# cheshmi/parsy_bench

Measured on AMD Instinct MI355X. Metric: Cholesky factorizations/sec (+ SpTRSV solves/sec), SuiteSparse SPD set, higher is better.
Workload: dtype f64; 1 GPU; flan-class stand-in (BASELINE.json configs[2] when flan: Flan_1565): grid (116, 116, 116) 27-point stencil, geometric nested dissection; n=1560896, nnz_A_lower=21491316, nsuper=81191, nnz_L=2044454227, xsize=2421483055, etree_levels=17, launches_per_factorization=357, parallelism=1 GPU

## Files before the change

### parsy_bench_amd/csrc/capi_exec.hip

```cpp
#include <hip/hip_runtime.h>

#include <chrono>
#include <cstdio>
#include <cstring>
#include <map>
#include <algorithm>
#include <mutex>
#include <string>
#include <tuple>
#include <vector>

#include "../../include/parsy_amd.h"
#include "errors.hpp"
#include "hip_check.hpp"
#include "dist.hpp"
#include "executor.hpp"
#include "inspector.hpp"
#include "plan_util.hpp"
#include "refine.hpp"
#include "schedule_digest.hpp"
#include "cond.hpp"
#include "eigs.hpp"
#include "feature_states.hpp"

// ... 445 lines not shown
    const parsy::Schedule& S = pl->S;
    int64_t n = 0;
    int li = 0;
    for (const parsy::Launch& l : S.chol) {
        if (l.kind != parsy::kLaunchDense) continue;
        for (int q = l.first; q < l.first + l.count; ++q, ++n)
            if (out && n < cap) {
                out[2 * n] = li;
                out[2 * n + 1] = S.big_tasks[(size_t)q].part;
            }
        ++li;
    }
    return n;
}

int64_t parsy_debug_launches(const parsy_plan* pl, int which, int32_t* out, int64_t cap) {
    if (!pl || which < 0 || which > 2) return -1;
    const parsy::Schedule& S = pl->S;
    const std::vector<parsy::Launch>& seq = which == 0 ? S.chol : which == 1 ? S.solve : S.bsolve;
    for (size_t i = 0; out && i < seq.size() && (int64_t)i < cap; ++i) {
        const parsy::Launch& l = seq[i];
        const int32_t row[parsy::kLaunchFields] = {l.kind, l.first, l.count, l.level, l.side, l.wait_level, l.form, l.rows_only,
                                                   l.ticket, l.lds_bytes, l.stage, l.width, l.width_class, l.task_first, l.task_count};
        std::copy(row, row + parsy::kLaunchFields, out + (size_t)parsy::kLaunchFields * i);
    }
    return (int64_t)seq.size();
}

int parsy_debug_schedule_digest(const parsy_plan* pl, int field, uint64_t* out, const char** name) {
    if (!pl) return -1;
// ... 469 lines not shown
```

### parsy_bench_amd/csrc/chol_kernels.hip

```cpp
#include <hip/hip_runtime.h>

#include <algorithm>

#include <climits>

#include "device_util.hpp"
#include "kernels.hpp"

namespace parsy {

static constexpr int kThreads = 256;
static constexpr int kLdSub = kSub + 1;

#ifdef PARSY_BIGSTAMPS
__device__ unsigned long long g_bigtrace[2 * 8 * 1024];
__device__ int g_bigstamp_cfg[2];
#define BIGSTAMP(i) do { if (st_on) g_bigtrace[((size_t)st_slot * 1024 + st_n) * 8 + (i)] = __builtin_readcyclecounter(); } while (0)
#else
#define BIGSTAMP(i) do { } while (0)
#endif

#ifdef PARSY_STAMPS
__device__ unsigned long long g_stamps[32];
#define STAMP(i) do { if (threadIdx.x == 0) g_stamps[i] = wall_clock64(); } while (0)
// ... 1354 lines not shown
static constexpr int kBigThreads = 64 * kBigWaves;
static_assert(kBK % 4 == 0 && kBK % kBigWaves == 0, "k_chol_big: a wave stages kBK / waves columns per operand");
struct BigLds {
    double R[2][kBK * kBLd];
    double C[2][kBK * kBLd];
};

static constexpr int kGldsAux = 0;
__device__ __forceinline__ void glds16(const double* g, double* lds) {
    __builtin_amdgcn_global_load_lds((const __attribute__((address_space(1))) void*)g,
                                     (__attribute__((address_space(3))) void*)lds, 16, 0, kGldsAux);
}

__global__ __launch_bounds__(kBigThreads, 4) void k_chol_big(const SnDesc* __restrict__ sn,
                                                             const int32_t* __restrict__ relpos,
                                                             const WaveEntry* __restrict__ ents,
                                                             const TileDesc* __restrict__ tasks,
                                                             double* __restrict__ L) {
    __shared__ __attribute__((aligned(16))) BigLds S;
    {
        int agpr_hint = 0;
        asm volatile("; accumulators in AGPRs %0" ::"a"(agpr_hint));
    }
    const int tid = threadIdx.x, lane = tid & 63;
    const int wave = __builtin_amdgcn_readfirstlane(tid >> 6);
    const int l15 = lane & 15, kq = lane >> 4;
    const TileDesc td = tasks[blockIdx.x];
    const SnDesc D = sn[td.sn];
    double* __restrict__ G = L + D.px;
    const int ld = D.ld;
    const int64_t e_begin = td.wp, e_end = td.sp;
    if (e_begin >= e_end) return;
#ifdef PARSY_BIGABL_ZEROOPS
    const long long zmask = td.part == 12345 ? -1ll : 0ll;
#endif
#ifdef PARSY_BIGSTAMPS
    const bool st_on = (int)gridDim.x == g_bigstamp_cfg[0] && (int)blockIdx.x == g_bigstamp_cfg[1] && lane == 0 &&
                       (wave == 0 || wave == 5);
    const int st_slot = wave == 0 ? 0 : 1;
    int st_n = 0;
#endif

    int64_t le = e_begin;
    int lk = 0;
    WaveEntry LE = ents[le];
    int offR = 0, offC = 0;
    auto enter = [&]() {
// ... 601 lines not shown
    (void)hipMemcpyFromSymbol(out, HIP_SYMBOL(g_trace), sizeof(unsigned long long) * 16 * 512);
}
extern "C" void parsy_debug_tilephase(unsigned long long* out, int reset) {
    (void)hipMemcpyFromSymbol(out, HIP_SYMBOL(g_tilephase), sizeof(unsigned long long) * 16);
    if (reset) {
        unsigned long long z[16] = {};
        (void)hipMemcpyToSymbol(HIP_SYMBOL(g_tilephase), z, sizeof(z));
    }
}
#endif

void launch_chol_big(const DevicePattern& P, int first, int count, double* L, hipStream_t stream) {
    if (count <= 0) return;
    witness_launch(kWCholBig);
    hipLaunchKernelGGL(k_chol_big, dim3(count), dim3(kBigThreads), 0, stream, P.csn, P.relpos, P.big_entries,
                       P.big_tasks + first, L);
}

void launch_chol_tiles(const DevicePattern& P, int first, int count, double* L, hipStream_t stream) {
    if (count <= 0) return;
    witness_launch(kWCholTiles);
    hipLaunchKernelGGL(k_chol_tiles, dim3(count), dim3(kThreads), 0, stream, P.csn, P.relpos, P.wave_entries,
                       P.wave_ptr, P.split_ranges, P.tile_scratch, P.tiles + first, L);
}

int chain_workgroups_per_cu() {
    int nb = 0;
    if (hipOccupancyMaxActiveBlocksPerMultiprocessor(&nb, k_chol_chain, kThreads, 0) != hipSuccess) return 0;
    return nb;
}

// ... 18 lines not shown
```

### parsy_bench_amd/csrc/executor.hip

```cpp
#include "executor.hpp"

#include <climits>
#include <cstdlib>
#include <cstring>
#include <stdexcept>

#include "cond.hpp"
#include "device_util.hpp"
#include "errors.hpp"
#include "hip_check.hpp"
#include "plan_fwd.hpp"
#include "plan_util.hpp"
#include "refine.hpp"
#include "feature_states.hpp"

namespace parsy {

const Schedule& plan_schedule(const parsy_plan* plan) { return plan->S; }

int check_plan(const parsy_plan* pl, const char* who, PlanNeeds needs) {
    const std::string w(who);
    if (pl->device < 0) return set_last_error(w + ": plan was built without a device (device < 0)"), -1;
    if (needs == kNeedsDevice) return 0;
    if (pl->solve_only) return set_last_error(w + ": plan was built from L's pattern only (no A pattern)"), -1;
// ... 119 lines not shown
    return dptr ? 0 : pool_failed(pool);
}

int plan_upload_launches(parsy_plan* pl) {
    if (pl->device < 0) return 0;
    PARSY_HIP(hipSetDevice(pl->device));
    pl->launches.clear();
    pl->levels_open = false;
    const Schedule& S = pl->S;
    if (upload(pl, S.small_list, pl->dp.small_list, true)) return -1;
    if (upload(pl, S.small_ranges, pl->dp.small_ranges, true)) return -1;
    if (upload(pl, S.solve_small_ranges, pl->dp.solve_small_ranges, true)) return -1;
    if (upload(pl, S.bsolve_ranges, pl->dp.bsolve_ranges, true)) return -1;
    if (upload(pl, S.tiles, pl->dp.tiles, true)) return -1;
    if (upload(pl, S.big_tasks, pl->dp.big_tasks, true)) return -1;
    if (upload(pl, S.solve_small_list, pl->dp.solve_small_list, true)) return -1;
    if (upload(pl, S.solve_panels, pl->dp.solve_panels, true)) return -1;
    if (upload(pl, S.solve_mtasks, pl->dp.solve_mtasks, true)) return -1;
    if (upload(pl, S.solve_fix_list, pl->dp.solve_fix_list, true)) return -1;
    if (upload(pl, S.solve_wide_list, pl->dp.solve_wide_list, true)) return -1;
    if (upload(pl, S.bsolve_blocks, pl->dp.bsolve_blocks, true)) return -1;
    if (upload(pl, S.bsolve_below, pl->dp.bsolve_below, true)) return -1;
    (void)pl->bpart.reset();
    pl->dp.bpart = nullptr;
    if (upload(pl, S.bsolve_pairs, pl->dp.bsolve_pairs, true)) return -1;
    if (upload(pl, S.sub_members, pl->dp.sub_members, true) || upload(pl, S.sub_trees, pl->dp.sub_trees, true) ||
        upload(pl, S.sub_slots, pl->dp.sub_slots, true) || upload(pl, S.sub_out_rows, pl->dp.sub_out_rows, true))
        return -1;
    pl->dp.sub_ntiers = (!S.sub_tiers.empty() && solve_sub_prepare(S.sub_max_slots) == 0) ? (int)S.sub_tiers.size() : 0;
    {
// ... 568 lines not shown
```

### parsy_bench_amd/csrc/kernels.hpp

```cpp
#pragma once
#include <hip/hip_runtime.h>

#include <cstdint>

#include "schedule.hpp"

namespace parsy {

constexpr int kPassLanes = 8;

struct SolveGates {
    int mrhs_min = 6;
    int chain_mrhs_min = 2;
    int bmrhs_min = 16;
    bool bmrhs_wide_only = true;
    int bchain_min_blocks = 128;
    int small_halves_min = 512;
    int sub_mrhs_min = 6;
    int xt_min = 16;
    bool xt_min_set = false;
    int wait_bias = 0;
    int sub_abl = 0;
};
SolveGates read_solve_gates();
// ... 55 lines not shown
    const UpdDesc* upd = nullptr;
    const int32_t* relpos = nullptr;
    const int64_t* a_dst = nullptr;
    const int32_t* rows = nullptr;
    const WaveEntry* wave_entries = nullptr;
    const int64_t* wave_ptr = nullptr;
    const int64_t* split_ranges = nullptr;
    double* tile_scratch = nullptr;
    const int32_t* small_list = nullptr;
    const int32_t* small_ranges = nullptr;
    const int32_t* solve_small_ranges = nullptr;
    const int32_t* bsolve_ranges = nullptr;
    const TileDesc* tiles = nullptr;
    const WaveEntry* big_entries = nullptr;
    const TileDesc* big_tasks = nullptr;
    const int32_t* solve_small_list = nullptr;
    const PanelDesc* solve_panels = nullptr;
    const PanelDesc* solve_mtasks = nullptr;
    const int32_t* solve_fix_list = nullptr;
    const int32_t* solve_wide_list = nullptr;
    const PanelDesc* bsolve_pairs = nullptr;
    const PanelDesc* bsolve_below = nullptr;
    double* bpart = nullptr;
    const PanelDesc* bsolve_blocks = nullptr;
    const SubMember* sub_members = nullptr;
    const SubTree* sub_trees = nullptr;
    const uint16_t* sub_slots = nullptr;
    const int32_t* sub_out_rows = nullptr;
    int sub_ntiers = 0;
    int* info = nullptr;
// ... 68 lines not shown
```

### parsy_bench_amd/csrc/schedule.cpp

```cpp
#include "schedule.hpp"

#include <cstdio>
#include <map>
#include <algorithm>
#include <queue>
#include <climits>
#include <cmath>
#include <cstdlib>
#include <cstdint>
#include <functional>
#include <stdexcept>
#include <string>

namespace parsy {

static inline int ceil_div(int a, int b) { return (a + b - 1) / b; }

static int env_int(const char* name, int dflt) {
    const char* v = std::getenv(name);
    if (!v || !*v) return dflt;
    return std::atoi(v);
}

static int find_subtrees(const std::vector<int>& parent, const std::vector<uint8_t>& eligible,
// ... 671 lines not shown
                                              (int32_t)(launch >> 1), (int32_t)((launch & 1) == 0), bigk[i].sr, bigk[i].sc,
                                              (int64_t)mid, (int32_t)std::min<int64_t>(dweight, INT32_MAX),
                                              (int32_t)std::min<int64_t>(dchunks, INT32_MAX), nstrips});
        i = j;
    }
}

}

void build_schedule(const PatternRef& P, const size_t* lC, const int* A2p, const int* A2i,
                    const uint8_t* active, Schedule& S, int compute_units) {
    S = Schedule();
    BuildState B;
    B.knobs = read_build_knobs();
    B.compute_units = compute_units;
    if (compute_units > 0) S.walker_batch = std::max(4, std::min(kWalkerBatch, compute_units / 2));
    describe_supernodes(P, lC, A2p, S);
    list_updates(P, lC, A2p, A2i, S, B);
    choose_sizes(S, B.knobs);
    cut_pieces(P, S, B);
    describe_updates(S, B);
    cut_subtrees(S, B);
    choose_super_tiles(S, B);
    build_wave_streams(S, B);
    collect_big_entries(S, B);
    build_big_tasks(S, B);
    build_launches(S, active);
}


struct LaunchKnobs {
    bool force_unfused;
    int big_group;
    int chain_split;
    int bsolve_below;
    bool sub_tier_min_trees_set;
    int sub_tier_min_trees;
    int solve_one;
};

static LaunchKnobs read_launch_knobs(const Schedule& S) {
    LaunchKnobs K{};
    const char* fu = std::getenv("PARSY_FORCE_UNFUSED");
    K.force_unfused = fu && fu[0] == '1';
    K.big_group = env_int("PARSY_BIG_GROUP", kBigGroup);
    K.chain_split = env_int("PARSY_CHAIN_SPLIT", S.update_flops >= kChainSplitAutoFlops ? 2 : 0);
    K.bsolve_below = env_int("PARSY_BSOLVE_BELOW", 1);
    K.sub_tier_min_trees_set = std::getenv("PARSY_SUB_TIER_MIN_TREES") != nullptr;
    K.sub_tier_min_trees = env_int("PARSY_SUB_TIER_MIN_TREES", kSubTierMinTrees);
    K.solve_one = env_int("PARSY_SOLVE_ONE", 1);
    return K;
}

static void build_solve_one(Schedule& S, const LaunchKnobs& K, bool sharded);

static bool append_sub_tier(Schedule& S, const std::vector<std::vector<int32_t>>& trees, int top_level, int max_slots) {
    const size_t members0 = S.sub_members.size(), trees0 = S.sub_trees.size(), slots0 = S.sub_slots.size(),
                 outs0 = S.sub_out_rows.size();
    auto drop = [&] {
        S.sub_members.resize(members0);
        S.sub_trees.resize(trees0);
        S.sub_slots.resize(slots0);
        S.sub_out_rows.resize(outs0);
        return false;
    };
// ... 204 lines not shown
    L.task_first = task_first;
    return L;
}
static Launch fixup_launch(int32_t count, int32_t level) {
    Launch L = main_launch(kLaunchSolveFixup, 0, level);
    L.count = count;
    return L;
}
static Launch back_block_launch(int32_t first, int32_t count, int32_t level, int32_t width_class) {
    Launch L = main_launch(kLaunchBackBlock, first, level);
    L.count = count;
    L.width_class = width_class;
    return L;
}

namespace {

using BigTaskList = std::vector<const Schedule::BigTask*>;

struct LaunchState {
    LaunchKnobs knobs;
    std::vector<Launch> early;
    std::vector<size_t> level_begin;
    std::vector<BigTaskList> big_next, big_push;
};

void reset_launch_lists(Schedule& S) {
    S.n_chain_launches = 0;
    S.n_solve_chain_launches = 0;
    S.n_solve_wide = 0;
    S.n_bpart_slots = 0;
    S.small_list.clear();
    S.small_ranges.clear();
    S.tiles.clear();
    S.big_tasks.clear();
    S.chol.clear();
    S.solve_small_list.clear();
    S.solve_small_ranges.clear();
    S.solve_panels.clear();
    S.solve_mtasks.clear();
    S.solve_fix_list.clear();
    S.solve_wide_list.clear();
    S.solve.clear();
    S.sub_members.clear();
    S.sub_trees.clear();
    S.sub_slots.clear();
    S.sub_out_rows.clear();
    S.sub_tiers.clear();
    S.sub_max_slots = 0;
    S.sub_cover_level = -1;
// ... 17 lines not shown
        S.bsolve_subtree_all = S.bsolve_subtree;
    }
    S.solve_subtree = S.solve_subtree_all;
    S.bsolve_subtree = S.bsolve_subtree_all;
    if (active)
        for (auto* sub : {&S.solve_subtree, &S.bsolve_subtree}) {
            const int count = sub == &S.solve_subtree ? S.n_solve_subtrees : S.n_bsolve_subtrees;
            std::vector<uint8_t> whole((size_t)std::max(count, 0), 1);
            for (int t = 0; t < ns; ++t)
                if ((*sub)[t] >= 0 && !S.active[t]) whole[(size_t)(*sub)[t]] = 0;
            for (int t = 0; t < ns; ++t)
                if ((*sub)[t] >= 0 && !whole[(size_t)(*sub)[t]]) (*sub)[t] = -1;
        }
}

Launch emit_big(Schedule& S, int big_group, const BigTaskList& all, Launch L, bool dense) {
    BigTaskList v;
    for (const Schedule::BigTask* b : all)
        if (dense ? b->em > b->e0 : b->e1 > b->em) v.push_back(b);
    if (v.empty()) return L;
    L.first = (int32_t)S.big_tasks.size();
    auto wt = [dense](const Schedule::BigTask* b) { return dense ? b->dweight : b->weight; };
    auto desc = [dense](const Schedule::BigTask* b) {
        return dense ? TileDesc{b->sn, b->row0, b->col0, b->dchunks | (b->strips > 0 ? kDenseStripTask : 0), b->e0, b->em}
                     : TileDesc{b->sn, b->row0, b->col0, 0, b->em, b->e1};
    };
    auto by_weight = [&](const Schedule::BigTask* a, const Schedule::BigTask* b) { return wt(a) > wt(b); };
    int g = big_group;
    const int per_task = v[0]->sr * v[0]->sc;
    while (g > 1 && (int64_t)v.size() * per_task < (int64_t)8 * kBigGroupsPerXcd * g * g) g /= 2;
    if (g < std::max(v[0]->sr, v[0]->sc)) g = 1;
    if (g <= 1) {
        std::stable_sort(v.begin(), v.end(), by_weight);
        for (const Schedule::BigTask* b : v) S.big_tasks.push_back(desc(b));
// ... 54 lines not shown
    }
    size_t len = 0;
    for (int x = 0; x < 8; ++x) len = std::max(len, seq[x].size());
    for (size_t s = 0; s < len; ++s)
        for (int x = 0; x < 8; ++x) {
            if (s < seq[x].size()) {
                S.big_tasks.push_back(desc(seq[x][s]));
            } else {
                S.big_tasks.push_back(TileDesc{0, 0, 0, 0, 0, 0});
            }
        }
    L.count = (int32_t)(8 * len);
    return L;
}

template <class Position, class Append>
int32_t subtree_ranges(const Schedule& S, const std::vector<int32_t>& subtree, int count, const std::vector<double>& cost,
                       Position&& position, Append&& append, std::vector<int32_t>& ranges, bool chol = false) {
    std::vector<std::vector<int32_t>> members((size_t)count);
    std::vector<double> total((size_t)count, 0.0);
    for (int t = 0; t < S.nsuper; ++t)
        if (subtree[t] >= 0 && (chol ? S.active_piece[S.piece0[t]] : S.active[t])) {
            members[(size_t)subtree[t]].push_back(t);
            total[(size_t)subtree[t]] += cost[t];
        }
    std::vector<int32_t> order;
    for (int k = 0; k < count; ++k)
        if (!members[(size_t)k].empty()) order.push_back(k);
    std::stable_sort(order.begin(), order.end(), [&](int a, int b) { return total[(size_t)a] > total[(size_t)b]; });
    for (int k : order) {
// ... 21 lines not shown
            [&](int32_t t) { add_small(S, S.piece0[t], L); }, S.small_ranges, true);
        if (L.count > 0) S.chol.push_back(L);
    }
    Launch L = small_launch((int32_t)S.small_list.size(), lev);
    for (int q = S.clevelPtr[lev]; q < S.clevelPtr[lev + 1]; ++q) {
        const int t = S.clevelSet[q];
        if (!S.active_piece[t] || S.chol_subtree[S.csn_real[t]] >= 0) continue;
        if (is_small(S.csn[t])) add_small(S, t, L);
        else tiled.push_back(t);
    }
    L.count = (int32_t)S.small_list.size() - L.first;
    if (L.count > 0) S.chol.push_back(L);
}

void push_next_launches(Schedule& S, LaunchState& LS, int lev) {
    const int g = LS.knobs.big_group;
    if (lev + 2 < S.cnlevels) {
        Launch Ld = emit_big(S, g, LS.big_push[lev], side_launch(kLaunchDense, 0, lev + 2, lev), true);
        if (Ld.count > 0) LS.early.push_back(Ld);
        Launch Lp = emit_big(S, g, LS.big_push[lev], side_launch(kLaunchBig, 0, lev + 2, lev), false);
        if (Lp.count > 0) LS.early.push_back(Lp);
    }
    if (lev > 0) {
        Launch Ld = emit_big(S, g, LS.big_next[lev - 1], main_launch(kLaunchDense, 0, lev), true);
        if (Ld.count > 0) S.chol.push_back(Ld);
        Launch Ln = emit_big(S, g, LS.big_next[lev - 1], main_launch(kLaunchBig, 0, lev), false);
        if (Ln.count > 0) S.chol.push_back(Ln);
    }
}

void tiles_launch(Schedule& S, LaunchState& LS, int lev, const std::vector<int>& tiled) {
    Launch Lt = side_launch(kLaunchTiles, (int32_t)S.tiles.size(), lev, lev - 2);
    std::vector<std::pair<int32_t, TileDesc>> wt;
    for (int t : tiled) {
        const SnDesc& T = S.csn[t];
        const int nbc = ceil_div(T.w, kTile), nbr = ceil_div(T.r, kTile);
        const int32_t* tw = &S.tile_w[S.sn_tw0[t]];
        for (int J = 0; J < nbc; ++J)
            for (int I = J; I < nbr; ++I) {
                const int32_t wgt = tw[((size_t)J * nbr + I) * 2];
                if (wgt <= 0) continue;
                const int64_t si = S.tile_split[S.sn_tw0[t] / 2 + (size_t)J * nbr + I];
                if (si < 0) {
// ... 948 lines not shown
            if (u < 0 || mi < 1 || mi > kBigTile || nj < 1 || nj > kBigTile || E.ia + mi + ms > S.upd[u].m || E.ja + nj + ns > S.upd[u].n1 ||
                ident != (S.upd[u].rel < 0) || S.level_of[S.upd_src[u]] != b.src_level) {
                fail("BIG entry " + std::to_string(e) + " of piece " + std::to_string(b.sn) + " has a bad window or source");
                continue;
            }
            auto rel_at = [&](int k) { return ident ? k : S.relpos[(size_t)S.upd[u].rel + k] - T.rbias; };
            if (rel_at(E.ia) / win_r != b.row0 / win_r || rel_at(E.ia + mi + ms - 1) / win_r != b.row0 / win_r ||
                rel_at(E.ja) / win_c != b.col0 / win_c || rel_at(E.ja + nj + ns - 1) / win_c != b.col0 / win_c)
                fail("BIG entry " + std::to_string(e) + " names rows outside its task's tile");
            covered[(size_t)u] += block_flops(E);
        }
    }
    {
        std::vector<int64_t> starts;
        std::vector<int64_t> dense_pos(S.big_all.size(), -1), ragged_pos(S.big_all.size(), -1);
        int64_t li = 0;
        for (const Launch& l : S.chol) {
            ++li;
            if (l.kind != kLaunchBig && l.kind != kLaunchDense) continue;
            const bool dense = l.kind == kLaunchDense;
            const bool side = l.side != 0;
            auto find_task = [&](int64_t e) -> const Schedule::BigTask* {
                auto it = std::upper_bound(S.big_all.begin(), S.big_all.end(), e,
                                           [](int64_t v, const Schedule::BigTask& b) { return v < b.e0; });
                if (it == S.big_all.begin()) return nullptr;
                --it;
                return e < it->e1 ? &*it : nullptr;
            };
            auto right_launch = [&](const Schedule::BigTask& b) {
                return side != (b.next != 0) && (side ? l.wait_level : l.level - 1) == b.src_level;
            };
            for (int q = l.first; q < l.first + l.count; ++q) {
                const TileDesc& td = S.big_tasks[(size_t)q];
                if (td.wp >= td.sp) {
                    if (td.wp != td.sp) fail("BIG launch task " + std::to_string(q) + " has a negative entry range");
                    continue;
                }
                const Schedule::BigTask* it = find_task(td.wp);
                const bool ok = it && (dense ? (it->e0 == td.wp && it->em == td.sp && (td.part & ~kDenseStripTask) == it->dchunks &&
                                                ((td.part & kDenseStripTask) != 0) == (it->strips > 0))
                                             : (it->em == td.wp && it->e1 == td.sp));
                if (!ok || it->sn != td.sn || it->row0 != td.row0 || it->col0 != td.col0) {
                    fail("BIG launch task " + std::to_string(q) + " is not a task of the plan");
                    continue;
                }
                if (!right_launch(*it)) fail("BIG launch task " + std::to_string(q) + " runs in the launch of another source level");
                (dense ? dense_pos : ragged_pos)[(size_t)(it - S.big_all.data())] = li;
                starts.push_back(td.wp);
            }
        }
        std::sort(starts.begin(), starts.end());
        if (std::adjacent_find(starts.begin(), starts.end()) != starts.end()) fail("a BIG task is launched twice");
        int64_t want = 0;
        for (size_t k = 0; k < S.big_all.size(); ++k) {
            const Schedule::BigTask& b = S.big_all[k];
            if (b.em < b.e0 || b.em > b.e1) fail("BIG task " + std::to_string(k) + " has a bad dense / ragged split");
            int64_t dch = 0;
            int32_t nst = 0;
            for (int64_t e = b.e0; e < b.em; ++e) {
                const WaveEntry& E = S.big_entries[(size_t)e];
                nst += big_strip_rows(E) || big_strip_cols(E);
                if (E.K < kDenseChunk) fail("BIG entry " + std::to_string(e) + " is filed as dense but is narrower than a chunk");
                dch += ceil_div(E.K, kDenseChunk);
            }
            if (dch != b.dchunks) fail("BIG task " + std::to_string(k) + " has a wrong dense chunk count");
            if (nst != b.strips) fail("BIG task " + std::to_string(k) + " has a wrong count of entries with strips");
            if (!S.active_piece[b.sn]) continue;
            want += (b.em > b.e0) + (b.e1 > b.em);
            if (b.em > b.e0 && b.e1 > b.em && !(dense_pos[k] > 0 && ragged_pos[k] > dense_pos[k]))
                fail("BIG task " + std::to_string(k) + ": the ragged part is not launched after the dense part");
        }
        if ((int64_t)starts.size() != want)
            fail("BIG launches hold " + std::to_string(starts.size()) + " task parts, the active targets have " + std::to_string(want));
    }
    for (int t = 0; t < nc; ++t) {
        const SnDesc& T = S.csn[t];
        if (is_small(T)) continue;
        for (int64_t u = T.upd0; u < T.upd0 + T.nupd; ++u) {
            const UpdDesc& U = S.upd[u];
            const double want = (double)U.K * U.n1 * (U.n1 + 1) + 2.0 * U.K * (double)(U.m - U.n1) * U.n1;
            if (std::abs(covered[(size_t)u] - want) > 1e-9 * want + 0.5)
                fail("update " + std::to_string(u) + " of piece " + std::to_string(t) + " is not covered exactly once by its entries");
// ... 55 lines not shown
```

### parsy_bench_amd/csrc/schedule.hpp

```cpp
#pragma once
#include <cstddef>
#include <cstdint>
#include <string>
#include <vector>

#include "inspector.hpp"

namespace parsy {

constexpr int kTile = 64;
constexpr int kSub = 32;
constexpr int kSmallMaxEntries = 6144;
constexpr int kSmallMaxWidth = 64;
constexpr int kBelowRows = 512;
constexpr int kBelowMaxGroups = 512;
constexpr int kBackGroup = 2;
constexpr int kTinyWidth = 16;
constexpr int kTinyWidth2 = 32;
constexpr int kPanelRows = 128;
constexpr int kSolveRows = 256;
constexpr int kSolveRowsMrhs = 128;

struct SnDesc {
    int64_t px;
// ... 19 lines not shown

struct WaveEntry {
    int64_t src;
    int32_t rel;
    int32_t ld, K;
    int32_t ia, ja;
    int32_t mn;
};
constexpr int kStripMax = 16;
inline int entry_rows(const WaveEntry& E) { return E.mn & 255; }
inline int entry_cols(const WaveEntry& E) { return (E.mn >> 8) & 255; }
inline bool big_ident(const WaveEntry& E) { return (E.mn >> 16) & 1; }
inline int big_strip_rows(const WaveEntry& E) { return (E.mn >> 17) & 31; }
inline int big_strip_cols(const WaveEntry& E) { return (E.mn >> 22) & 31; }
constexpr int kDenseStripTask = 1 << 30;

struct TileDesc {
    int32_t sn;
    int32_t row0, col0;
    int32_t part;
    int64_t wp;
    int64_t sp;
};

struct PanelDesc {
    int32_t sn;
    int32_t jb;
    int32_t row0;
    int32_t pad;
};
// ... 66 lines not shown
constexpr int kBigTile = 128;
constexpr int kBigMinK = 128;
constexpr int kPieceWidth = 512;
constexpr double kBigAutoFlops = 1e11;
constexpr double kPieceAutoFlops = 2e12;
constexpr double kChainSplitAutoFlops = 1e11;
constexpr int kBigSuperMinTasks = 12288;
constexpr double kBigSuperMaxFill = 0.85;
constexpr int kBigGroup = 8;
constexpr int kBigGroupsPerXcd = 2;
constexpr int kBigTailGroups = 16;
constexpr int kDenseChunk = 8;
constexpr double kDenseMinShare = 0.25;
constexpr double kDenseMinFill = 0.70;
constexpr double kDenseAllShare = 0.06;
constexpr int kPushGroup = 1;
constexpr int kOneMaxSupernodes = 8192;
constexpr int64_t kOneLargeEntries = 4096;
constexpr int64_t kOneMaxEntries = 1 << 28;
constexpr int kOneMaxSupernodesBig = 32768;
constexpr int kOneSmallBlocks = 1024;
constexpr int kOneMidBlocks = 4096;
constexpr int kOneRhs8Density = 300;
constexpr int kOneMaxRhs = 8;
constexpr int kCholSubtreesPerCu = 64;
constexpr int kSubtreesPerCu = 16;
constexpr double kSubtreeMinCost = 2e5;
constexpr int kSubtreeMinPerSlot = 2;
constexpr int kSolveSubtreeMinMembers = 2048;

struct Schedule {
    int n = 0, nsuper = 0, nlevels = 0;
    bool solve_only = false;
    int64_t nnzA = 0, ssize = 0, xsize = 0, nnzL = 0;
    int max_width = 0, max_rows = 0, n_small = 0, n_big = 0;
    int n_solve_wide = 0;
    int64_t n_dslots = 0;
    int64_t n_tflags = 0;
    int n_chain_launches = 0;
    int n_solve_chain_launches = 0;
    int walker_batch = kWalkerBatch;
    double flops_stored = 0, update_flops = 0, reread_bytes = 0;
    double tile_update_flops = 0;
    double inner_flops = 0;

    std::vector<SnDesc> sn;
    std::vector<int> sparent;
    std::vector<SnDesc> csn;
    std::vector<int32_t> piece0;
    std::vector<int32_t> csn_real;
    std::vector<int> clevelPtr, clevelSet;
    int cnlevels = 0;
    int big_min_k = kBigMinK, piece_width = kPieceWidth, push_group = kPushGroup;
    int big_super_r = 0, big_super_c = 0;
    std::vector<UpdDesc> upd;
// ... 14 lines not shown
    std::vector<uint16_t> sub_slots;
    std::vector<int32_t> sub_out_rows;
    std::vector<SubTier> sub_tiers;
    int sub_cover_level = -1;
    int sub_max_slots = 0;

    std::vector<int32_t> small_list;
    std::vector<TileDesc> tiles;
    std::vector<WaveEntry> big_entries;
    struct BigTask { int32_t sn, row0, col0, weight; int64_t e0, e1; int32_t src_level, next;
                     int32_t sr, sc;
                     int64_t em; int32_t dweight, dchunks;
                     int32_t strips; };
    std::vector<BigTask> big_all;
    std::vector<TileDesc> big_tasks;
    double big_flops = 0;
    double dense_flops = 0;
    int64_t n_dense_entries = 0;
    int64_t n_strip_entries = 0;
    std::vector<Launch> chol;

    std::vector<int32_t> solve_small_list;
    std::vector<PanelDesc> solve_panels;
    std::vector<PanelDesc> solve_mtasks;
    std::vector<int32_t> solve_fix_list;
    std::vector<int32_t> solve_wide_list;
    std::vector<Launch> solve;

    std::vector<PanelDesc> bsolve_pairs;
    std::vector<PanelDesc> bsolve_blocks;
// ... 23 lines not shown
    std::vector<int> levelPtr, levelSet;
    std::vector<int64_t> split_ranges;
    std::vector<int64_t> tile_split;
    struct SplitDesc { int64_t ranges; int64_t sp; int32_t nparts; int32_t pad; };
    std::vector<SplitDesc> split_desc;
    int64_t n_split_doubles = 0;
    std::vector<int64_t> sn_wp0;
    std::vector<int64_t> sn_tw0;
    std::vector<int32_t> tile_w;
    std::vector<int32_t> level_of;
};

void build_schedule(const PatternRef& P, const size_t* lC, const int* A2p, const int* A2i,
                    const uint8_t* active, Schedule& out, int compute_units = 0);
void build_launches(Schedule& S, const uint8_t* active, const uint8_t* active_pieces = nullptr);
int64_t simulate_chain(const Schedule& S, int slots);
int64_t check_schedule(const Schedule& S, std::string& what);
constexpr int kSmallMaxUpdates = 8;
inline bool is_small(const SnDesc& d) {
    return d.w <= kSmallMaxWidth && (int64_t)d.w * d.r <= kSmallMaxEntries && d.nupd <= kSmallMaxUpdates;
}

}
```

### parsy_bench_amd/csrc/schedule_digest.hpp

```cpp
#pragma once
#include <cstdint>
#include <cstring>
#include <type_traits>
#include <utility>
#include <vector>

#include "schedule.hpp"

namespace parsy {

struct Fnv1a {
    uint64_t h = 14695981039346656037ULL;
    void bytes(const void* p, size_t n) {
        const unsigned char* b = static_cast<const unsigned char*>(p);
        for (size_t i = 0; i < n; ++i) h = (h ^ b[i]) * 1099511628211ULL;
    }
    template <class T>
    void value(const T& v) {
        static_assert(std::is_arithmetic_v<T>, "digest: a scalar is an integer, a bool or a double");
        if constexpr (std::is_same_v<T, bool>) {
            const unsigned char b = v ? 1 : 0;
            bytes(&b, 1);
        } else {
            unsigned char raw[sizeof(T)];
// ... 9 lines not shown
    void vec(const std::vector<T>& v) {
        const uint64_t len = v.size();
        value(len);
        if constexpr (std::is_same_v<T, Schedule::BigTask>) {
            for (const T& x : v) value(x);
        } else {
            static_assert(std::is_same_v<T, double> || std::has_unique_object_representations_v<T>,
                          "digest: this element type has padding -- hash it member by member");
            if (!v.empty()) bytes(v.data(), v.size() * sizeof(T));
        }
    }
};

using ScheduleDigest = std::vector<std::pair<const char*, uint64_t>>;

static_assert(sizeof(Schedule) == 1968,
              "Schedule changed: list every data member in schedule_digest() (schedule_digest.hpp), then update this size");
static_assert(sizeof(Schedule::OneLists) == 176,
              "Schedule::OneLists changed: list every data member in schedule_digest() (schedule_digest.hpp), then update this size");

inline ScheduleDigest schedule_digest(const Schedule& S, int only = -1) {
    ScheduleDigest out;
#define PARSY_DIGEST_SCALAR(m)                                \
    {                                                         \
        Fnv1a f;                                              \
        if (only < 0 || only == (int)out.size()) f.value(S.m); \
        out.push_back({#m, f.h});                             \
    }
#define PARSY_DIGEST_VECTOR(m)                              \
    {                                                       \
        Fnv1a f;                                            \
        if (only < 0 || only == (int)out.size()) f.vec(S.m); \
        out.push_back({#m, f.h});                           \
    }
#define PARSY_DIGEST_ONE(o)                                                                              \
    PARSY_DIGEST_VECTOR(o.sn) PARSY_DIGEST_VECTOR(o.slot0) PARSY_DIGEST_VECTOR(o.wleft) PARSY_DIGEST_SCALAR(o.nslots) \
    PARSY_DIGEST_VECTOR(o.pull_ptr) PARSY_DIGEST_VECTOR(o.pull_slot) PARSY_DIGEST_VECTOR(o.pull_pos) PARSY_DIGEST_VECTOR(o.member)
    PARSY_DIGEST_SCALAR(n) PARSY_DIGEST_SCALAR(nsuper) PARSY_DIGEST_SCALAR(nlevels) PARSY_DIGEST_SCALAR(solve_only)
    PARSY_DIGEST_SCALAR(nnzA) PARSY_DIGEST_SCALAR(ssize) PARSY_DIGEST_SCALAR(xsize) PARSY_DIGEST_SCALAR(nnzL)
    PARSY_DIGEST_SCALAR(max_width) PARSY_DIGEST_SCALAR(max_rows) PARSY_DIGEST_SCALAR(n_small) PARSY_DIGEST_SCALAR(n_big)
    PARSY_DIGEST_SCALAR(n_solve_wide) PARSY_DIGEST_SCALAR(n_dslots) PARSY_DIGEST_SCALAR(n_tflags)
    PARSY_DIGEST_SCALAR(n_chain_launches) PARSY_DIGEST_SCALAR(n_solve_chain_launches) PARSY_DIGEST_SCALAR(walker_batch)
    PARSY_DIGEST_SCALAR(flops_stored) PARSY_DIGEST_SCALAR(update_flops) PARSY_DIGEST_SCALAR(reread_bytes)
    PARSY_DIGEST_SCALAR(tile_update_flops) PARSY_DIGEST_SCALAR(inner_flops)
    PARSY_DIGEST_VECTOR(sn) PARSY_DIGEST_VECTOR(sparent)
    PARSY_DIGEST_VECTOR(csn) PARSY_DIGEST_VECTOR(piece0) PARSY_DIGEST_VECTOR(csn_real)
    PARSY_DIGEST_VECTOR(clevelPtr) PARSY_DIGEST_VECTOR(clevelSet) PARSY_DIGEST_SCALAR(cnlevels)
    PARSY_DIGEST_SCALAR(big_min_k) PARSY_DIGEST_SCALAR(piece_width) PARSY_DIGEST_SCALAR(push_group)
    PARSY_DIGEST_SCALAR(big_super_r) PARSY_DIGEST_SCALAR(big_super_c)
    PARSY_DIGEST_VECTOR(upd) PARSY_DIGEST_VECTOR(upd_src) PARSY_DIGEST_VECTOR(relpos) PARSY_DIGEST_VECTOR(a_dst)
    PARSY_DIGEST_VECTOR(rows) PARSY_DIGEST_VECTOR(wave_entries) PARSY_DIGEST_VECTOR(wave_ptr)
    PARSY_DIGEST_VECTOR(chol_subtree) PARSY_DIGEST_VECTOR(solve_subtree) PARSY_DIGEST_VECTOR(bsolve_subtree)
    PARSY_DIGEST_VECTOR(solve_subtree_all) PARSY_DIGEST_VECTOR(bsolve_subtree_all)
    PARSY_DIGEST_VECTOR(chol_cost) PARSY_DIGEST_VECTOR(solve_cost)
    PARSY_DIGEST_SCALAR(n_chol_subtrees) PARSY_DIGEST_SCALAR(n_solve_subtrees) PARSY_DIGEST_SCALAR(n_bsolve_subtrees)
    PARSY_DIGEST_VECTOR(small_ranges) PARSY_DIGEST_VECTOR(solve_small_ranges) PARSY_DIGEST_VECTOR(bsolve_ranges)
    PARSY_DIGEST_VECTOR(sub_members) PARSY_DIGEST_VECTOR(sub_trees) PARSY_DIGEST_VECTOR(sub_slots)
    PARSY_DIGEST_VECTOR(sub_out_rows) PARSY_DIGEST_VECTOR(sub_tiers)
    PARSY_DIGEST_SCALAR(sub_cover_level) PARSY_DIGEST_SCALAR(sub_max_slots)
    PARSY_DIGEST_VECTOR(small_list) PARSY_DIGEST_VECTOR(tiles)
    PARSY_DIGEST_VECTOR(big_entries) PARSY_DIGEST_VECTOR(big_all) PARSY_DIGEST_VECTOR(big_tasks)
    PARSY_DIGEST_SCALAR(big_flops) PARSY_DIGEST_SCALAR(dense_flops)
    PARSY_DIGEST_SCALAR(n_dense_entries) PARSY_DIGEST_SCALAR(n_strip_entries)
    PARSY_DIGEST_VECTOR(chol)
    PARSY_DIGEST_VECTOR(solve_small_list) PARSY_DIGEST_VECTOR(solve_panels) PARSY_DIGEST_VECTOR(solve_mtasks)
    PARSY_DIGEST_VECTOR(solve_fix_list) PARSY_DIGEST_VECTOR(solve_wide_list) PARSY_DIGEST_VECTOR(solve)
    PARSY_DIGEST_VECTOR(bsolve_pairs) PARSY_DIGEST_VECTOR(bsolve_blocks) PARSY_DIGEST_VECTOR(bsolve_below)
    PARSY_DIGEST_SCALAR(n_bpart_slots) PARSY_DIGEST_VECTOR(bsolve)
    PARSY_DIGEST_SCALAR(solve_one) PARSY_DIGEST_SCALAR(solve_one_back) PARSY_DIGEST_SCALAR(one_subtrees)
    PARSY_DIGEST_SCALAR(one_big) PARSY_DIGEST_SCALAR(one_forced)
    PARSY_DIGEST_ONE(one_f)
    PARSY_DIGEST_ONE(one_b)
    PARSY_DIGEST_VECTOR(active) PARSY_DIGEST_VECTOR(active_piece) PARSY_DIGEST_VECTOR(chol_level_begin)
    PARSY_DIGEST_VECTOR(levelPtr) PARSY_DIGEST_VECTOR(levelSet)
    PARSY_DIGEST_VECTOR(split_ranges) PARSY_DIGEST_VECTOR(tile_split) PARSY_DIGEST_VECTOR(split_desc)
    PARSY_DIGEST_SCALAR(n_split_doubles)
// ... 9 lines not shown
```

Before: 2.974 factorizations/s.

## Split tail-round dense big tiles into 64x64 sub-window tasks in the big kernel

Dense big tasks that fill a single full tile (one entry, K at or above a threshold) are taken out of the dense launch and re-emitted as 64x64 sub-window tasks in the ragged big launch. Windows lying entirely above the diagonal are skipped. A cost model built from constant timings (T1 tail, T4, gap) decides when to cut: either a small launch that fits in one round, or the partial last round of a larger launch. The goal is to fill idle CUs during the tail wave. In exchange it adds schedule bookkeeping, a second entry array passed to the kernel, and new validation checks.

New measurement: 2.969 factorizations/s, median of 2. About the same (-0.2%).

```diff
diff --git a/parsy_bench_amd/csrc/capi_exec.hip b/parsy_bench_amd/csrc/capi_exec.hip
--- a/parsy_bench_amd/csrc/capi_exec.hip
+++ b/parsy_bench_amd/csrc/capi_exec.hip
@@ -483,6 +483,39 @@
     return n;
 }
 
+int64_t parsy_debug_fit_tasks(const parsy_plan* pl, int32_t* out, int64_t cap, int64_t* counts) {
+    if (!pl) return -1;
+    const parsy::Schedule& S = pl->S;
+    if (counts) {
+        counts[0] = S.n_fit_eligible;
+        counts[1] = S.n_fit_cut;
+        counts[2] = S.n_fit_skipped;
+        counts[3] = S.dense_slots;
+    }
+    int64_t n = 0;
+    for (size_t li = 0; li < S.chol.size(); ++li) {
+        const parsy::Launch& l = S.chol[li];
+        if (l.kind != parsy::kLaunchBig) continue;
+        for (int q = l.first; q < l.first + l.count; ++q) {
+            const parsy::TileDesc& td = S.big_tasks[(size_t)q];
+            if (td.part != parsy::kBigFitTask || td.wp >= td.sp) continue;
+            if (out && n < cap) {
+                const parsy::WaveEntry& W = S.fit_entries[(size_t)td.wp];
+                int32_t* o = out + 7 * n;
+                o[0] = (int32_t)li;
+                o[1] = S.fit_parent[(size_t)td.wp];
+                o[2] = W.K;
+                o[3] = parsy::entry_rows(W);
+                o[4] = parsy::entry_cols(W);
+                o[5] = W.ia;
+                o[6] = W.ja;
+            }
+            ++n;
+        }
+    }
+    return n;
+}
+
 int64_t parsy_debug_launches(const parsy_plan* pl, int which, int32_t* out, int64_t cap) {
     if (!pl || which < 0 || which > 2) return -1;
     const parsy::Schedule& S = pl->S;
diff --git a/parsy_bench_amd/csrc/chol_kernels.hip b/parsy_bench_amd/csrc/chol_kernels.hip
--- a/parsy_bench_amd/csrc/chol_kernels.hip
+++ b/parsy_bench_amd/csrc/chol_kernels.hip
@@ -1392,7 +1392,8 @@
 
 __global__ __launch_bounds__(kBigThreads, 4) void k_chol_big(const SnDesc* __restrict__ sn,
                                                              const int32_t* __restrict__ relpos,
-                                                             const WaveEntry* __restrict__ ents,
+                                                             const WaveEntry* __restrict__ big_ents,
+                                                             const WaveEntry* __restrict__ fit_ents,
                                                              const TileDesc* __restrict__ tasks,
                                                              double* __restrict__ L) {
     __shared__ __attribute__((aligned(16))) BigLds S;
@@ -1409,6 +1410,7 @@
     const int ld = D.ld;
     const int64_t e_begin = td.wp, e_end = td.sp;
     if (e_begin >= e_end) return;
+    const WaveEntry* __restrict__ ents = td.part == kBigFitTask ? fit_ents : big_ents;
 #ifdef PARSY_BIGABL_ZEROOPS
     const long long zmask = td.part == 12345 ? -1ll : 0ll;
 #endif
@@ -2040,7 +2042,7 @@
     if (count <= 0) return;
     witness_launch(kWCholBig);
     hipLaunchKernelGGL(k_chol_big, dim3(count), dim3(kBigThreads), 0, stream, P.csn, P.relpos, P.big_entries,
-                       P.big_tasks + first, L);
+                       P.fit_entries, P.big_tasks + first, L);
 }
 
 void launch_chol_tiles(const DevicePattern& P, int first, int count, double* L, hipStream_t stream) {
diff --git a/parsy_bench_amd/csrc/executor.hip b/parsy_bench_amd/csrc/executor.hip
--- a/parsy_bench_amd/csrc/executor.hip
+++ b/parsy_bench_amd/csrc/executor.hip
@@ -157,6 +157,7 @@
     if (upload(pl, S.bsolve_ranges, pl->dp.bsolve_ranges, true)) return -1;
     if (upload(pl, S.tiles, pl->dp.tiles, true)) return -1;
     if (upload(pl, S.big_tasks, pl->dp.big_tasks, true)) return -1;
+    if (upload(pl, S.fit_entries, pl->dp.fit_entries, true)) return -1;
     if (upload(pl, S.solve_small_list, pl->dp.solve_small_list, true)) return -1;
     if (upload(pl, S.solve_panels, pl->dp.solve_panels, true)) return -1;
     if (upload(pl, S.solve_mtasks, pl->dp.solve_mtasks, true)) return -1;
diff --git a/parsy_bench_amd/csrc/kernels.hpp b/parsy_bench_amd/csrc/kernels.hpp
--- a/parsy_bench_amd/csrc/kernels.hpp
+++ b/parsy_bench_amd/csrc/kernels.hpp
@@ -93,6 +93,7 @@
     const TileDesc* tiles = nullptr;
     const WaveEntry* big_entries = nullptr;
     const TileDesc* big_tasks = nullptr;
+    const WaveEntry* fit_entries = nullptr;
     const int32_t* solve_small_list = nullptr;
     const PanelDesc* solve_panels = nullptr;
     const PanelDesc* solve_mtasks = nullptr;
diff --git a/parsy_bench_amd/csrc/schedule.cpp b/parsy_bench_amd/csrc/schedule.cpp
--- a/parsy_bench_amd/csrc/schedule.cpp
+++ b/parsy_bench_amd/csrc/schedule.cpp
@@ -2,6 +2,7 @@
 
 #include <cstdio>
 #include <map>
+#include <set>
 #include <algorithm>
 #include <queue>
 #include <climits>
@@ -709,6 +710,7 @@
     BuildState B;
     B.knobs = read_build_knobs();
     B.compute_units = compute_units;
+    if (compute_units > 0) S.dense_slots = 2 * compute_units;
     if (compute_units > 0) S.walker_batch = std::max(4, std::min(kWalkerBatch, compute_units / 2));
     describe_supernodes(P, lC, A2p, S);
     list_updates(P, lC, A2p, A2i, S, B);
@@ -732,6 +734,7 @@
     bool sub_tier_min_trees_set;
     int sub_tier_min_trees;
     int solve_one;
+    int big_fit;
 };
 
 static LaunchKnobs read_launch_knobs(const Schedule& S) {
@@ -744,6 +747,7 @@
     K.sub_tier_min_trees_set = std::getenv("PARSY_SUB_TIER_MIN_TREES") != nullptr;
     K.sub_tier_min_trees = env_int("PARSY_SUB_TIER_MIN_TREES", kSubTierMinTrees);
     K.solve_one = env_int("PARSY_SOLVE_ONE", 1);
+    K.big_fit = env_int("PARSY_BIG_FIT", 1);
     return K;
 }
 
@@ -978,9 +982,17 @@
     return L;
 }
 
+bool fit_eligible(const Schedule& S, const Schedule::BigTask& b) {
+    if (b.e1 - b.e0 != 1 || b.em != b.e1 || b.sr != 1 || b.sc != 1 || b.strips != 0) return false;
+    const WaveEntry& E = S.big_entries[(size_t)b.e0];
+    return big_ident(E) && entry_rows(E) == kBigTile && entry_cols(E) == kBigTile && big_strip_rows(E) == 0 &&
+           big_strip_cols(E) == 0;
+}
+
 namespace {
 
 using BigTaskList = std::vector<const Schedule::BigTask*>;
+using FitCuts = std::set<const Schedule::BigTask*>;
 
 struct LaunchState {
     LaunchKnobs knobs;
@@ -998,6 +1010,9 @@
     S.small_ranges.clear();
     S.tiles.clear();
     S.big_tasks.clear();
+    S.fit_entries.clear();
+    S.fit_parent.clear();
+    S.n_fit_eligible = S.n_fit_cut = S.n_fit_skipped = 0;
     S.chol.clear();
     S.solve_small_list.clear();
     S.solve_small_ranges.clear();
@@ -1045,10 +1060,10 @@
         }
 }
 
-Launch emit_big(Schedule& S, int big_group, const BigTaskList& all, Launch L, bool dense) {
+Launch emit_big(Schedule& S, int big_group, const BigTaskList& all, Launch L, bool dense, const FitCuts* cuts = nullptr) {
     BigTaskList v;
     for (const Schedule::BigTask* b : all)
-        if (dense ? b->em > b->e0 : b->e1 > b->em) v.push_back(b);
+        if (dense ? b->em > b->e0 && !(cuts && cuts->count(b)) : b->e1 > b->em) v.push_back(b);
     if (v.empty()) return L;
     L.first = (int32_t)S.big_tasks.size();
     auto wt = [dense](const Schedule::BigTask* b) { return dense ? b->dweight : b->weight; };
@@ -1133,6 +1148,69 @@
     return L;
 }
 
+FitCuts fit_cuts(Schedule& S, int mode, const BigTaskList& all, const Launch& Ld) {
+    FitCuts cuts;
+    if (Ld.count <= 0) return cuts;
+    std::map<int64_t, const Schedule::BigTask*> by_e0;
+    for (const Schedule::BigTask* b : all)
+        if (b->em > b->e0) by_e0[b->e0] = b;
+    BigTaskList eligible;
+    int64_t T = 0;
+    for (int q = Ld.first; q < Ld.first + Ld.count; ++q) {
+        const TileDesc& td = S.big_tasks[(size_t)q];
+        if (td.wp >= td.sp) continue;
+        ++T;
+        const Schedule::BigTask* b = by_e0.at(td.wp);
+        if (fit_eligible(S, *b)) eligible.push_back(b);
+    }
+    const int64_t Te = (int64_t)eligible.size();
+    S.n_fit_eligible += Te;
+    if (mode == 0 || Te == 0) return cuts;
+    const int slots = S.dense_slots;
+    if (mode >= 2) {
+        for (int64_t q = 0; q < std::min<int64_t>(Te, slots); ++q) cuts.insert(eligible[(size_t)q]);
+        return cuts;
+    }
+    const int K = S.big_entries[(size_t)eligible[0]->e0].K;
+    for (const Schedule::BigTask* b : eligible)
+        if (S.big_entries[(size_t)b->e0].K != K) return cuts;
+    if (K < kFitMinK) return cuts;
+    const int64_t one_round = slots / 4;
+    if (Te == T && T <= one_round) {
+        if (kFitT4Us < kFitT1TailUs) cuts.insert(eligible.begin(), eligible.end());
+    } else if (T > slots && (T - Te) * 8 <= T) {
+        const int64_t r = T % slots;
+        if (r > 0 && r <= std::min(one_round, Te) && kFitT4Us + kFitGapUs < kFitT1TailUs) cuts.insert(eligible.end() - r, eligible.end());
+    }
+    return cuts;
+}
+
+void append_fit_tasks(Schedule& S, const BigTaskList& all, const FitCuts& cuts, Launch& Lb) {
+    if (cuts.empty()) return;
+    if (Lb.count == 0) Lb.first = (int32_t)S.big_tasks.size();
+    for (const Schedule::BigTask* b : all) {
+        if (!cuts.count(b)) continue;
+        const WaveEntry& E = S.big_entries[(size_t)b->e0];
+        ++S.n_fit_cut;
+        for (int dj = 0; dj < kBigTile; dj += kFitEdge)
+            for (int di = 0; di < kBigTile; di += kFitEdge) {
+                if (E.ia + di + kFitEdge - 1 < E.ja + dj) {
+                    ++S.n_fit_skipped;
+                    continue;
+                }
+                WaveEntry W = E;
+                W.ia += di;
+                W.ja += dj;
+                W.mn = kFitEdge | (kFitEdge << 8) | (1 << 16);
+                const int64_t at = (int64_t)S.fit_entries.size();
+                S.fit_entries.push_back(W);
+                S.fit_parent.push_back((int32_t)(b - S.big_all.data()));
+                S.big_tasks.push_back(TileDesc{b->sn, b->row0, b->col0, kBigFitTask, at, at + 1});
+                ++Lb.count;
+            }
+    }
+}
+
 template <class Position, class Append>
 int32_t subtree_ranges(const Schedule& S, const std::vector<int32_t>& subtree, int count, const std::vector<double>& cost,
                        Position&& position, Append&& append, std::vector<int32_t>& ranges, bool chol = false) {
@@ -1184,19 +1262,23 @@
 }
 
 void push_next_launches(Schedule& S, LaunchState& LS, int lev) {
-    const int g = LS.knobs.big_group;
-    if (lev + 2 < S.cnlevels) {
-        Launch Ld = emit_big(S, g, LS.big_push[lev], side_launch(kLaunchDense, 0, lev + 2, lev), true);
-        if (Ld.count > 0) LS.early.push_back(Ld);
-        Launch Lp = emit_big(S, g, LS.big_push[lev], side_launch(kLaunchBig, 0, lev + 2, lev), false);
-        if (Lp.count > 0) LS.early.push_back(Lp);
-    }
-    if (lev > 0) {
-        Launch Ld = emit_big(S, g, LS.big_next[lev - 1], main_launch(kLaunchDense, 0, lev), true);
-        if (Ld.count > 0) S.chol.push_back(Ld);
-        Launch Ln = emit_big(S, g, LS.big_next[lev - 1], main_launch(kLaunchBig, 0, lev), false);
-        if (Ln.count > 0) S.chol.push_back(Ln);
-    }
+    auto emit_pair = [&](const BigTaskList& all, const Launch& dense_proto, const Launch& big_proto, std::vector<Launch>& out) {
+        const int g = LS.knobs.big_group;
+        const size_t mark = S.big_tasks.size();
+        Launch Ld = emit_big(S, g, all, dense_proto, true);
+        const FitCuts cuts = fit_cuts(S, LS.knobs.big_fit, all, Ld);
+        if (!cuts.empty()) {
+            S.big_tasks.resize(mark);
+            Ld = emit_big(S, g, all, dense_proto, true, &cuts);
+        }
+        if (Ld.count > 0) out.push_back(Ld);
+        Launch Lb = emit_big(S, g, all, big_proto, false);
+        append_fit_tasks(S, all, cuts, Lb);
+        if (Lb.count > 0) out.push_back(Lb);
+    };
+    if (lev + 2 < S.cnlevels)
+        emit_pair(LS.big_push[lev], side_launch(kLaunchDense, 0, lev + 2, lev), side_launch(kLaunchBig, 0, lev + 2, lev), LS.early);
+    if (lev > 0) emit_pair(LS.big_next[lev - 1], main_launch(kLaunchDense, 0, lev), main_launch(kLaunchBig, 0, lev), S.chol);
 }
 
 void tiles_launch(Schedule& S, LaunchState& LS, int lev, const std::vector<int>& tiled) {
@@ -2175,6 +2257,7 @@
     {
         std::vector<int64_t> starts;
         std::vector<int64_t> dense_pos(S.big_all.size(), -1), ragged_pos(S.big_all.size(), -1);
+        std::vector<uint8_t> fit_cover(S.big_all.size(), 0);
         int64_t li = 0;
         for (const Launch& l : S.chol) {
             ++li;
@@ -2197,6 +2280,34 @@
                     if (td.wp != td.sp) fail("BIG launch task " + std::to_string(q) + " has a negative entry range");
                     continue;
                 }
+                if (!dense && td.part == kBigFitTask) {
+                    const int64_t f = td.wp;
+                    if (td.sp != f + 1 || f < 0 || f >= (int64_t)S.fit_entries.size() || S.fit_parent.size() != S.fit_entries.size() ||
+                        S.fit_parent[(size_t)f] < 0 || S.fit_parent[(size_t)f] >= (int32_t)S.big_all.size()) {
+                        fail("sub-window task " + std::to_string(q) + " has a bad entry or parent");
+                        continue;
+                    }
+                    const size_t k = (size_t)S.fit_parent[(size_t)f];
+                    const Schedule::BigTask& b = S.big_all[k];
+                    const WaveEntry& W = S.fit_entries[(size_t)f];
+                    if (!fit_eligible(S, b) || !S.active_piece[b.sn] || b.sn != td.sn || b.row0 != td.row0 || b.col0 != td.col0) {
+                        fail("sub-window task " + std::to_string(q) + ": its parent may not be cut");
+                        continue;
+                    }
+                    const WaveEntry& E = S.big_entries[(size_t)b.e0];
+                    const int di = W.ia - E.ia, dj = W.ja - E.ja, mi = entry_rows(W), nj = entry_cols(W);
+                    const bool window_ok = (di == 0 || di == kFitEdge) && (dj == 0 || dj == kFitEdge) && mi == kFitEdge && nj == kFitEdge;
+                    if (!window_ok || W.src != E.src || W.ld != E.ld || W.K != E.K || W.rel != E.rel || !big_ident(W) || (W.mn >> 17) != 0 ||
+                        W.ia + mi - 1 < W.ja) {
+                        fail("sub-window task " + std::to_string(q) + " is not a window of its parent's entry");
+                        continue;
+                    }
+                    if (!right_launch(b)) fail("sub-window task " + std::to_string(q) + " runs in the launch of another source level");
+                    const uint8_t bit = (uint8_t)(1 << (2 * (di / kFitEdge) + dj / kFitEdge));
+                    if (fit_cover[k] & bit) fail("sub-window tasks of BIG task " + std::to_string(k) + " overlap");
+                    fit_cover[k] |= bit;
+                    continue;
+                }
                 const Schedule::BigTask* it = find_task(td.wp);
                 const bool ok = it && (dense ? (it->e0 == td.wp && it->em == td.sp && (td.part & ~kDenseStripTask) == it->dchunks &&
                                                 ((td.part & kDenseStripTask) != 0) == (it->strips > 0))
@@ -2227,6 +2338,16 @@
             if (dch != b.dchunks) fail("BIG task " + std::to_string(k) + " has a wrong dense chunk count");
             if (nst != b.strips) fail("BIG task " + std::to_string(k) + " has a wrong count of entries with strips");
             if (!S.active_piece[b.sn]) continue;
+            if (fit_cover[k]) {
+                if (dense_pos[k] > 0) fail("BIG task " + std::to_string(k) + " runs as a dense task and as sub-window tasks");
+                const WaveEntry& E = S.big_entries[(size_t)b.e0];
+                uint8_t need = 0;
+                for (int a = 0; a < 2; ++a)
+                    for (int c = 0; c < 2; ++c)
+                        if (E.ia + kFitEdge * a + kFitEdge - 1 >= E.ja + kFitEdge * c) need |= (uint8_t)(1 << (2 * a + c));
+                if (fit_cover[k] != need) fail("the sub-window tasks of BIG task " + std::to_string(k) + " do not tile its lower part");
+                continue;
+            }
             want += (b.em > b.e0) + (b.e1 > b.em);
             if (b.em > b.e0 && b.e1 > b.em && !(dense_pos[k] > 0 && ragged_pos[k] > dense_pos[k]))
                 fail("BIG task " + std::to_string(k) + ": the ragged part is not launched after the dense part");
diff --git a/parsy_bench_amd/csrc/schedule.hpp b/parsy_bench_amd/csrc/schedule.hpp
--- a/parsy_bench_amd/csrc/schedule.hpp
+++ b/parsy_bench_amd/csrc/schedule.hpp
@@ -57,6 +57,7 @@
 inline int big_strip_rows(const WaveEntry& E) { return (E.mn >> 17) & 31; }
 inline int big_strip_cols(const WaveEntry& E) { return (E.mn >> 22) & 31; }
 constexpr int kDenseStripTask = 1 << 30;
+constexpr int kBigFitTask = 1;
 
 struct TileDesc {
     int32_t sn;
@@ -153,6 +154,13 @@
 constexpr double kDenseMinShare = 0.25;
 constexpr double kDenseMinFill = 0.70;
 constexpr double kDenseAllShare = 0.06;
+constexpr int kFitEdge = 64;
+constexpr double kFitT1Us = 145.0;
+constexpr double kFitT1TailUs = 89.0;
+constexpr double kFitT4Us = 66.0;
+constexpr double kFitGapUs = 12.0;
+constexpr int kFitMinK = 512;
+constexpr int kFitHostCus = 256;
 constexpr int kPushGroup = 1;
 constexpr int kOneMaxSupernodes = 8192;
 constexpr int64_t kOneLargeEntries = 4096;
@@ -178,6 +186,7 @@
     int64_t n_tflags = 0;
     int n_chain_launches = 0;
     int n_solve_chain_launches = 0;
+    int dense_slots = 2 * kFitHostCus;
     int walker_batch = kWalkerBatch;
     double flops_stored = 0, update_flops = 0, reread_bytes = 0;
     double tile_update_flops = 0;
@@ -222,6 +231,11 @@
                      int32_t strips; };
     std::vector<BigTask> big_all;
     std::vector<TileDesc> big_tasks;
+    std::vector<WaveEntry> fit_entries;
+    std::vector<int32_t> fit_parent;
+    int64_t n_fit_eligible = 0;
+    int64_t n_fit_cut = 0;
+    int64_t n_fit_skipped = 0;
     double big_flops = 0;
     double dense_flops = 0;
     int64_t n_dense_entries = 0;
@@ -275,6 +289,7 @@
 void build_schedule(const PatternRef& P, const size_t* lC, const int* A2p, const int* A2i,
                     const uint8_t* active, Schedule& out, int compute_units = 0);
 void build_launches(Schedule& S, const uint8_t* active, const uint8_t* active_pieces = nullptr);
+bool fit_eligible(const Schedule& S, const Schedule::BigTask& b);
 int64_t simulate_chain(const Schedule& S, int slots);
 int64_t check_schedule(const Schedule& S, std::string& what);
 constexpr int kSmallMaxUpdates = 8;
diff --git a/parsy_bench_amd/csrc/schedule_digest.hpp b/parsy_bench_amd/csrc/schedule_digest.hpp
--- a/parsy_bench_amd/csrc/schedule_digest.hpp
+++ b/parsy_bench_amd/csrc/schedule_digest.hpp
@@ -47,7 +47,7 @@
 
 using ScheduleDigest = std::vector<std::pair<const char*, uint64_t>>;
 
-static_assert(sizeof(Schedule) == 1968,
+static_assert(sizeof(Schedule) == 2040,
               "Schedule changed: list every data member in schedule_digest() (schedule_digest.hpp), then update this size");
 static_assert(sizeof(Schedule::OneLists) == 176,
               "Schedule::OneLists changed: list every data member in schedule_digest() (schedule_digest.hpp), then update this size");
@@ -73,7 +73,7 @@
     PARSY_DIGEST_SCALAR(nnzA) PARSY_DIGEST_SCALAR(ssize) PARSY_DIGEST_SCALAR(xsize) PARSY_DIGEST_SCALAR(nnzL)
     PARSY_DIGEST_SCALAR(max_width) PARSY_DIGEST_SCALAR(max_rows) PARSY_DIGEST_SCALAR(n_small) PARSY_DIGEST_SCALAR(n_big)
     PARSY_DIGEST_SCALAR(n_solve_wide) PARSY_DIGEST_SCALAR(n_dslots) PARSY_DIGEST_SCALAR(n_tflags)
-    PARSY_DIGEST_SCALAR(n_chain_launches) PARSY_DIGEST_SCALAR(n_solve_chain_launches) PARSY_DIGEST_SCALAR(walker_batch)
+    PARSY_DIGEST_SCALAR(n_chain_launches) PARSY_DIGEST_SCALAR(n_solve_chain_launches) PARSY_DIGEST_SCALAR(dense_slots) PARSY_DIGEST_SCALAR(walker_batch)
     PARSY_DIGEST_SCALAR(flops_stored) PARSY_DIGEST_SCALAR(update_flops) PARSY_DIGEST_SCALAR(reread_bytes)
     PARSY_DIGEST_SCALAR(tile_update_flops) PARSY_DIGEST_SCALAR(inner_flops)
     PARSY_DIGEST_VECTOR(sn) PARSY_DIGEST_VECTOR(sparent)
@@ -93,6 +93,8 @@
     PARSY_DIGEST_SCALAR(sub_cover_level) PARSY_DIGEST_SCALAR(sub_max_slots)
     PARSY_DIGEST_VECTOR(small_list) PARSY_DIGEST_VECTOR(tiles)
     PARSY_DIGEST_VECTOR(big_entries) PARSY_DIGEST_VECTOR(big_all) PARSY_DIGEST_VECTOR(big_tasks)
+    PARSY_DIGEST_VECTOR(fit_entries) PARSY_DIGEST_VECTOR(fit_parent)
+    PARSY_DIGEST_SCALAR(n_fit_eligible) PARSY_DIGEST_SCALAR(n_fit_cut) PARSY_DIGEST_SCALAR(n_fit_skipped)
     PARSY_DIGEST_SCALAR(big_flops) PARSY_DIGEST_SCALAR(dense_flops)
     PARSY_DIGEST_SCALAR(n_dense_entries) PARSY_DIGEST_SCALAR(n_strip_entries)
     PARSY_DIGEST_VECTOR(chol)
```
